# rail-berkeley/serl

Hardware: AMD Instinct MI355X
Metric: learner grad-steps/sec (DrQ, bs256, 2x128x128 img) (higher is better)
Workload: dtype f32 (trunk convs as split-fp16 MFMA x3, fp32 accumulate; <=1e-6 vs fp64)

## Files before the change

serl_amd/csrc/agent.hip:

```cpp
#include <algorithm>
#include <cmath>
#include <cstdlib>
#include <cstring>
#include <string>
#include <vector>

#include "heads.h"
#include "small_encoder.h"

using namespace serl;

namespace {

struct CamOff { long sle, dW, db, lng, lnb, conv; };
struct Offs {
  CamOff cam[SERL_MAX_CAMS];
  long cam_stride;
  long c_w1, c_b1, c_g1, c_be1, c_w2, c_b2, c_g2, c_be2, c_hw, c_hb;
  long p_W, p_b, p_g, p_be;
  long a_w1, a_b1, a_g1, a_be1, a_w2, a_b2, a_g2, a_be2, a_Wm, a_bm, a_Ws, a_bs;
  long lam;
  long P, Pc, Pa0, Pa1;
};

// ... 1223 lines not shown
  const TrunkPlan& p = a->tws.plan;
  std::string s = "images=" + std::to_string(p.images) + " pool=" + std::to_string(p.pool) + " raw_b0=" + std::to_string(p.raw_b0);
  static const char* kNames[3] = {"conv0", "conv1", "proj"};
  for (int i = 0; i < kTrunkStages; ++i)
    for (int k = 0; k < 3; ++k) {
      const TrunkPlan::L& l = p.conv[i][k];
      if (!l.kern) continue;
      s += " b" + std::to_string(i) + "_" + kNames[k] + "=" + std::string(1, l.kern) + "/" + std::to_string(l.cfg) + "/" +
           std::to_string(l.pmode) + "/f" + std::to_string(l.fused) + "/p" + std::to_string(l.pad) + "x" + std::to_string(l.padw);
    }
  SERL_REQUIRE((int)s.size() < cap, "the plan text takes %d bytes, the buffer holds %d", (int)s.size() + 1, cap);
  snprintf(out, cap, "%s", s.c_str());
  return SERL_OK;
}

int serl_agent_debug_get(serl_agent* a, const char* what, float* host_out, int64_t count) {
  SERL_REQUIRE(a && what && host_out, "NULL argument");
  SERL_HIP(hipSetDevice(a->cfg.device));
  const Offs& o = a->o;
  const std::string w(what);
  const float* p = nullptr;
  long n = 0;
  const serl_agent_cfg& c = a->cfg;
  if (w == "ctr_nonzero") {
    SERL_REQUIRE(count == 1, "tap 'ctr_nonzero' holds one value");
    SERL_HIP(hipDeviceSynchronize());
    std::vector<int> h((size_t)kCtrPerLane * kCtrLanes);
    SERL_HIP(hipMemcpy(h.data(), a->ctr, sizeof(int) * h.size(), hipMemcpyDeviceToHost));
    long nz = 0;
    for (int v : h) nz += v != 0;
    host_out[0] = (float)nz;
    return SERL_OK;
  }
  if (w == "g_critic") { p = a->Gc; n = o.Pc; }
  else if (w == "g_actor") { p = a->Ga; n = o.Pa1 - o.Pa0; }
  else if (w == "scalars") { p = a->SC; n = kScalars; }
  else if (w == "q") { p = a->crit.q; n = (long)c.ensemble * c.batch; }
  else if (w == "q_target") { p = a->critT.q; n = (long)c.ensemble * c.batch; }
  else if (w == "target_q") { p = a->ytgt; n = c.batch; }
  else if (w == "x") { p = a->crit.x; n = (long)c.batch * a->XA; }
  else if (w == "x_target") { p = a->critT.x; n = (long)c.batch * a->XA; }
  else if (w == "feats") { p = a->feats; n = 2L * c.n_cam * c.batch * a->HW * 512; }
  else if (w == "logp") { p = a->pol.logp; n = c.batch; }
  else if (w == "dx") { p = a->dx; n = (long)c.batch * a->XA; }
  else { set_error("unknown debug tap '%s'", what); return SERL_ERR_INVALID; }
  SERL_REQUIRE(count <= n && count > 0, "tap '%s' holds %ld floats, asked for %lld", what, n, (long long)count);
  SERL_HIP(hipDeviceSynchronize());
  SERL_HIP(hipMemcpy(host_out, p, sizeof(float) * count, hipMemcpyDeviceToHost));
  return SERL_OK;
}

int serl_agent_debug_set(serl_agent* a, const char* what, const float* host, int64_t count) {
  SERL_REQUIRE(a && what && host, "NULL argument");
  SERL_HIP(hipSetDevice(a->cfg.device));
  const Offs& o = a->o;
  const std::string w(what);
  float* p = nullptr;
  long n = 0;
  if (w == "g_critic") { p = a->Gc; n = o.Pc; }
  else if (w == "g_actor") { p = a->Ga; n = o.Pa1 - o.Pa0; }
  else if (w == "scalars") { p = a->SC; n = kScalars; }
  else { set_error("unknown debug tap '%s'", what); return SERL_ERR_INVALID; }
  SERL_REQUIRE(count <= n && count > 0, "tap '%s' holds %ld floats, got %lld", what, n, (long long)count);
  SERL_HIP(hipDeviceSynchronize());
  SERL_HIP(hipMemcpy(p, host, sizeof(float) * count, hipMemcpyHostToDevice));
  if (a->last_global <= 0) a->last_global = 1;
  return SERL_OK;
}

// ... 2 lines not shown
```

serl_amd/csrc/trunk.hip:

```cpp
#include <algorithm>

#include "internal.h"
#include "prof.h"
#include "trunk_common.h"

namespace serl {

struct ConvInitArgs {
  const uint8_t* img;
  const float* w;
  float* out;
  double* stats;
  int N, H, W, Ho, Wo, tiles_y, tiles_x;
};

constexpr int kCiPatch = 37;
constexpr int kCiPW = kCiPatch * 3 + 2;
constexpr int kCiK = 148;
constexpr int kCiBS = 64 + 4;

__global__ __launch_bounds__(256) void conv_init_kernel(ConvInitArgs a) {
  extern __shared__ __attribute__((aligned(16))) float smem[];
  float* patch = smem;
  float* wl = smem + kCiPatch * kCiPW + 3;
// ... 516 lines not shown
  uint8_t* b = (uint8_t*)mem;
  size_t off = 0;
  for (int i = 0; i < kTrunkStages; ++i)
    for (int k = 0; k < 3; ++k) {
      if (k == 2 && i == 0) continue;
      int K, Cout;
      conv_dims(i, k, K, Cout);
      p.blk[i][k].hi = (uint16_t*)(b + off); off += al256((size_t)K * Cout * 2);
      p.blk[i][k].lo = (uint16_t*)(b + off); off += al256((size_t)K * Cout * 2);
      p.blk[i][k].inv = (float*)(b + off); off += al256((size_t)Cout * 4);
      p.blk[i][k].dma = nullptr;
      if (dma_copy(i, k)) { p.blk[i][k].dma = (uint16_t*)(b + off); off += al256((size_t)2 * K * Cout * 2); }
    }
  p.init.hi = (uint16_t*)(b + off); off += al256((size_t)64 * 224 * 2);
  p.init.lo = (uint16_t*)(b + off); off += al256((size_t)64 * 224 * 2);
  p.init.inv = (float*)(b + off); off += al256(64 * 4);
  p.zero = b + off; off += 256;
  p.dirty = true;
  return SERL_OK;
}

static int trunk_pack(const TrunkWeights& w, TrunkPacked& p, hipStream_t stream) {
  for (int i = 0; i < kTrunkStages; ++i)
    for (int k = 0; k < 3; ++k) {
      const float* src = k == 0 ? w.blk[i].conv0 : (k == 1 ? w.blk[i].conv1 : w.blk[i].proj);
      if (!src) continue;
      int K, Cout;
      conv_dims(i, k, K, Cout);
      int rc = pack_conv_weights_f16x3(src, p.blk[i][k].hi, p.blk[i][k].lo, p.blk[i][k].inv, K, Cout, stream);
      if (rc) return rc;
      if (p.blk[i][k].dma && (rc = pack_dma_order_f16x3(p.blk[i][k].hi, p.blk[i][k].lo, p.blk[i][k].dma, K, Cout, stream))) return rc;
    }
  {
    int rc = pack_conv_init_f16x3(w.conv_init, p.init.hi, p.init.lo, p.init.inv, stream);
    if (rc) return rc;
  }
  p.dirty = false;
  return SERL_OK;
}

int trunk_forward(const TrunkWeights& w, TrunkWorkspace& ws, const uint8_t* frames, int n, float* feats_out,
                  hipStream_t stream, TrunkPacked* packed, int stage_begin, int stage_end) {
  if (packed && packed->dirty) {
    int prc = trunk_pack(w, *packed, stream);
    if (prc) return prc;
  }
  if (packed) {
    SERL_REQUIRE(n > 0 && n <= ws.max_images, "trunk_forward: %d images exceeds workspace (%d)", n, ws.max_images);
    return trunk_forward_f16x3(w, ws, *packed, frames, n, feats_out, stream, stage_begin, stage_end);
  }
  SERL_REQUIRE(stage_begin < 0 && stage_end == kTrunkStages - 1, "the exact-fp32 trunk runs whole passes only");
  SERL_REQUIRE(n > 0 && n <= ws.max_images, "trunk_forward: %d images exceeds workspace (%d)", n, ws.max_images);
  const TrunkDims& d = ws.d;
  const int N = n;
  auto stats_of = [&](int layer) { return ws.stats + (size_t)layer * ws.max_images * kGnGroups * 2; };
  SERL_HIP(hipMemsetAsync(ws.stats, 0, (size_t)kGnLayers * ws.max_images * kGnGroups * 2 * sizeof(double), stream));
  int rc;
  {
    ConvInitArgs a{};
    a.img = frames; a.w = w.conv_init; a.out = ws.raw_init; a.stats = stats_of(0);
    a.N = N; a.H = d.H; a.W = d.W; a.Ho = d.h[0]; a.Wo = d.w[0];
    a.tiles_y = cd(a.Ho, 16); a.tiles_x = cd(a.Wo, 16);
    const size_t lds = (size_t)(kCiPatch * kCiPW + 3 + kCiK * kCiBS) * 4;
    ProfScope prof("conv_init", stream);
    hipLaunchKernelGGL(conv_init_kernel, dim3(N * a.tiles_y * a.tiles_x), dim3(256), lds, stream, a);
    SERL_HIP(hipGetLastError());
  }
// ... 41 lines not shown
```

serl_amd/csrc/trunk_common.h:

```cpp
#pragma once
#include "internal.h"

namespace serl {

typedef float f32x16 __attribute__((ext_vector_type(16)));

__device__ __forceinline__ int pool_pad_lo(int in, int out) { return max((out - 1) * 2 + 3 - in, 0) >> 1; }

__device__ __forceinline__ int xcd_remap(int b, int nwg) {
  const int q = nwg >> 3, r = nwg & 7, xcd = b & 7;
  return (xcd < r ? xcd * (q + 1) : r * (q + 1) + (xcd - r) * q) + (b >> 3);
}

__device__ __forceinline__ void stats_flush(float s, float q, double* stats_ng ,
                                            int chan, int gsize, bool valid, bool wait = true) {
#pragma unroll
  for (int off = 1; off < 16; off <<= 1) {
    s += __shfl_xor(s, off);
    q += __shfl_xor(q, off);
  }
  s += __shfl_xor(s, 32);
  q += __shfl_xor(q, 32);
  const int lane = threadIdx.x & 63;
  if (valid && (lane & 15) == 0 && lane < 32) {
// ... 30 lines not shown

__device__ __forceinline__ void gn_coef4(const GnRef& g, int n, int c, float4& sc, float4& sh) {
  const double* st = g.stats + ((size_t)n * kGnGroups + c / g.gsize) * 2;
  const double mean = st[0] * g.inv_count, m2 = st[1] * g.inv_count;
  const float var = fmaxf((float)(m2 - mean * mean), 0.f);
  const float rstd = rsqrtf(var + 1e-5f), mf = (float)mean;
  const float4 ga = *reinterpret_cast<const float4*>(g.gamma + c);
  const float4 be = *reinterpret_cast<const float4*>(g.beta + c);
  sc = make_float4(ga.x * rstd, ga.y * rstd, ga.z * rstd, ga.w * rstd);
  sh = make_float4(be.x - mf * sc.x, be.y - mf * sc.y, be.z - mf * sc.z, be.w - mf * sc.w);
}

struct ConvArgs {
  const float* in;
  const float* w;
  float* out;
  double* stats;
  GnRef in_gn;
  int N, Hi, Wi, Cin, Ho, Wo, Cout, KH, KW, stride, pad, padw;
  int M, P, tiles_m, tiles_n;
};

struct PackedConvWeights {
  const uint16_t* hi;
  const uint16_t* lo;
  const float* inv;
  const uint16_t* dma = nullptr;
};
int pack_conv_weights_f16x3(const float* w, uint16_t* hi, uint16_t* lo, float* inv, int K, int Cout, hipStream_t stream);
int pack_dma_order_f16x3(const uint16_t* hi, const uint16_t* lo, uint16_t* dma, int K, int Cout, hipStream_t stream);
int trunk_forward_f16x3(const TrunkWeights& w, TrunkWorkspace& ws, TrunkPacked& pk, const uint8_t* frames, int N,
                        float* feats_out, hipStream_t stream, int stage_begin = -1, int stage_end = kTrunkStages - 1);

int pack_conv_init_f16x3(const float* w, uint16_t* hi, uint16_t* lo, float* inv, hipStream_t stream);
int launch_conv_init_f16x3(const uint8_t* img, PackedConvWeights w, float* out, double* stats, int N, int H, int W,
                           int Ho, int Wo, hipStream_t stream, const float* pool_gamma = nullptr, int* ticket = nullptr,
                           bool complete_pool = false);

}
```

serl_amd/csrc/trunk_f16x3.hip:

```cpp
#include "trunk_f16x3_elementwise.h"

namespace serl {

static int resident_workgroups(hipStream_t stream) {
  thread_local hipStream_t last = nullptr;
  thread_local int last_n = -1;
  if (last_n >= 0 && last == stream) return last_n;
  int dev = 0, n = 0;
  hipDeviceProp_t prop;
  if (hipGetDevice(&dev) == hipSuccess && hipGetDeviceProperties(&prop, dev) == hipSuccess) n = prop.multiProcessorCount;
  uint32_t mask[16] = {0};
  if (hipExtStreamGetCUMask(stream, 16, mask) == hipSuccess) {
    int m = 0;
    for (uint32_t w : mask) m += __builtin_popcount(w);
    if (m > 0 && (n == 0 || m < n)) n = m;
  } else {
    (void)hipGetLastError();
  }
  last = stream; last_n = n;
  return n;
}

static_assert(kStageFilters[0] % 64 == 0 && kStageFilters[1] % 64 == 0 && kStageFilters[2] % 64 == 0 && kStageFilters[3] % 64 == 0,
              "conv channels unsupported (Cin % 32, Cout % 64)");
// ... 28 lines not shown
  const bool dma_ok = (cfg == 0 || cfg == 4) && a.Cin % 32 == 0 && zero_page && dma && fits32;
  if (slab_ok) {
    l.kern = 'S'; l.cfg = 9; l.raw = raw;
    const int tiles_n = a.Cout / 64;
    if (fuse && a.P % 256 == 0 && fused_can_wait(resident, a.P / 256 * tiles_n)) {
      l.fused = 1; l.expected = a.P / 256; l.group = a.P / 256 * tiles_n;
    }
    l.stagger = (l.fused && a.M / 256 * tiles_n >= 1024) ? 5 : 0;
  } else if (dma_ok) {
    l.kern = 'D'; l.cfg = cfg;
    const int tn = cfg == 0 ? 2 : 1, tiles_n = a.Cout / (64 * tn);
    if (pmode == 1 && cfg == 4) pmode = 3;
    if (fuse && pmode == 0 && a.P % 128 == 0 && tiles_n <= kSyncPerImage && fused_can_wait(resident, a.P / 128 * tiles_n)) {
      l.fused = 1; l.expected = a.P / 128; l.group = a.P / 128 * tiles_n;
    } else if (fuse && pmode == 0 && a.P == 64 && a.M % 128 == 0 && tn == 2 && a.Cout / kGnGroups == 64) {
      l.fused = 2;
    } else if (fuse && pmode == 2 && a.P == 16 && a.M % 128 == 0 && tn == 2 && a.Cout / kGnGroups == 128) {
      l.fused = 2;
    }
    l.proj = proj && pmode != 3 && a.KH == 3 && a.stride == 2 && a.pad == 0 && a.padw == 0;
  } else {
    l.kern = 'R'; l.cfg = cfg;
  }
  l.pmode = pmode;
  l.pad = a.pad; l.padw = a.padw;
  return l;
}

static int plan_pass(TrunkPlan& p, const TrunkDims& d, int N, const TrunkPacked& pk, const bool (&has_proj)[kTrunkStages], int resident,
                     bool fuse, bool proj_fuse) {
  p = TrunkPlan{};
  p.images = N; p.fuse = fuse;
  const bool fuse_pool = d.h[0] % 16 == 0 && d.w[0] % 16 == 0;
  const bool complete_pool = fuse_pool && N >= 512 && N % 512 == 0;
  p.pool = complete_pool ? 2 : (fuse_pool ? 1 : 0);
  const ConvArgs b0 = conv_geom(d, N, 0, 0);
  p.raw_b0 = complete_pool && fuse && !has_proj[0] && rowslab_shape_ok(b0) && b0.Cin <= 128 && pk.blk[0][0].dma && pk.blk[0][1].dma &&
             b0.P % 256 == 0 && fused_can_wait(resident, b0.P / 256 * (b0.Cout / 64));
  for (int i = 0; i < kTrunkStages; ++i) {
    TrunkPlan::L* l = p.conv[i];
    const bool raw = i == 0 && p.raw_b0;
    l[0] = plan_conv(conv_geom(d, N, i, 0), pk.blk[i][0].dma, pk.zero, fuse, resident, raw, has_proj[i] && proj_fuse && pk.blk[i][2].dma);
    if (l[0].proj) {
      l[2] = l[0];
      l[2].kern = 'F'; l[2].fused = 0;
    } else if (has_proj[i]) {
      l[2] = plan_conv(conv_geom(d, N, i, 2), pk.blk[i][2].dma, pk.zero, false, resident, false, false);
    }
    l[1] = plan_conv(conv_geom(d, N, i, 1), pk.blk[i][1].dma, pk.zero, fuse, resident, false, false);
    SERL_REQUIRE(!raw || (l[0].kern == 'S' && l[0].fused && l[1].fused),
                 "block 0 was planned on the fused row-slab path");
  }
  return SERL_OK;
}

template <int WM, int WN, int TM, int TN, int DEEP>
static void launch_igemm(ConvArgsB ab, int pmode, hipStream_t stream) {
  constexpr int BM = 32 * TM * WM, BN = 32 * TN * WN;
  ab.c.tiles_m = cdiv(ab.c.M, BM); ab.c.tiles_n = ab.c.Cout / BN;
  const dim3 grid(ab.c.tiles_m * ab.c.tiles_n), block(256);
  const size_t lds = (size_t)2 * (2 * BM * 64 + 2 * BN * 64);
  if (pmode == 0) hipLaunchKernelGGL((conv_igemm_f16x3_kernel<WM, WN, TM, TN, 0, DEEP>), grid, block, lds, stream, ab);
  else if (pmode == 1) hipLaunchKernelGGL((conv_igemm_f16x3_kernel<WM, WN, TM, TN, 1, DEEP>), grid, block, lds, stream, ab);
  else if (pmode == 2) hipLaunchKernelGGL((conv_igemm_f16x3_kernel<WM, WN, TM, TN, 2, DEEP>), grid, block, lds, stream, ab);
  else hipLaunchKernelGGL((conv_igemm_f16x3_kernel<WM, WN, TM, TN, 3, DEEP>), grid, block, lds, stream, ab);
}
template <int TN, bool PROJ>
// ... 76 lines not shown
                        float* feats_out, hipStream_t stream, int stage_begin, int stage_end) {
  const TrunkDims& d = ws.d;
  const TrunkPlan& plan = ws.plan;
  auto stats_of = [&](int layer) { return ws.stats + (size_t)layer * ws.max_images * kGnGroups * 2; };
  int rc;
  if (stage_begin < 0) {
    const char* gf = getenv("SERL_GN_FUSE");
    const char* pf = getenv("SERL_PROJ_FUSE");
    const bool fuse = !(gf && gf[0] == '0') && claim_fused_pass(stream);
    const bool has_proj[kTrunkStages] = {w.blk[0].proj != nullptr, w.blk[1].proj != nullptr, w.blk[2].proj != nullptr,
                                         w.blk[3].proj != nullptr};
    const int resident = fuse ? resident_workgroups(stream) : 0;
    if ((rc = plan_pass(ws.plan, d, N, pk, has_proj, resident, fuse, !(pf && pf[0] == '0')))) return rc;
    if (ws.stats_sync_bytes % 16 == 0 && ws.stats_sync_bytes < ((size_t)1 << 31)) {
      const long n16 = (long)(ws.stats_sync_bytes / 16);
      hipLaunchKernelGGL(zero_sys_kernel, dim3((unsigned)std::min<long>(cdiv(n16, 256), 512)), dim3(256), 0, stream, (void*)ws.stats, n16);
      SERL_HIP(hipGetLastError());
    } else {
      SERL_HIP(hipMemsetAsync(ws.stats, 0, ws.stats_sync_bytes, stream));
    }
  } else {
    SERL_REQUIRE(plan.images == N, "trunk pass piece over %d images continues a pass planned for %d", N, plan.images);
  }
  auto fuse_of = [&](int layer, int mode) {
    FuseArgs f{};
    f.mode = mode;
    f.sync = ws.sync + (size_t)layer * ((size_t)ws.max_images * kSyncPerImage + kSyncTickets);
    f.ticket = f.sync + (size_t)ws.max_images * kSyncPerImage;
    return f;
  };
  const GnRef gn_init = gn_ref(stats_of(0), w.gn_init_s, w.gn_init_b, d.h[0] * d.w[0], 64);
  if (stage_begin < 0) {
    if ((rc = launch_conv_init_f16x3(frames, PackedConvWeights{pk.init.hi, pk.init.lo, pk.init.inv}, ws.raw_init, stats_of(0), N, d.H,
                                     d.W, d.h[0], d.w[0], stream, plan.pool ? w.gn_init_s : nullptr, fuse_of(0, 0).ticket,
                                     plan.pool == 2))) return rc;
    if (plan.raw_b0) {
    } else if (plan.pool == 2) {
      const long tot = (long)N * d.h[1] * d.w[1] * 16;
      ProfScope prof("gn_relu_maxpool", stream);
      hipLaunchKernelGGL(gn_relu_split_kernel, dim3(cdiv(tot, 256)), dim3(256), 0, stream, ws.raw_init, gn_init,
                         reinterpret_cast<uint4*>(ws.pool), N, d.h[1] * d.w[1], 64);
      SERL_HIP(hipGetLastError());
    } else if (plan.pool == 1) {
      const long tot = (long)N * d.h[1] * (d.w[1] / 4) * 16;
      const int ty = d.h[0] / 16, tx = d.w[0] / 16;
      const float* pooled = ws.raw_init;
      const float* frows = pooled + (size_t)N * d.h[1] * d.w[1] * 64;
      const float* fcols = frows + (size_t)N * ty * d.w[0] * 64;
      ProfScope prof("gn_relu_maxpool", stream);
      hipLaunchKernelGGL(pool_finish_split_kernel, dim3(cdiv(tot, 256)), dim3(256), 0, stream, pooled, frows, fcols, gn_init,
                         reinterpret_cast<uint4*>(ws.pool), N, d.h[0], d.w[0], ty, tx);
      SERL_HIP(hipGetLastError());
    } else {
      const long tot = (long)N * d.h[1] * d.w[1] * 16;
      ProfScope prof("gn_relu_maxpool", stream);
      hipLaunchKernelGGL(gn_relu_maxpool_split_kernel, dim3(cdiv(tot, 256)), dim3(256), 0, stream, ws.raw_init, gn_init,
                         reinterpret_cast<uint4*>(ws.pool), N, d.h[0], d.w[0], d.h[1], d.w[1], 64);
      SERL_HIP(hipGetLastError());
    }
  }
  auto run_stage = [&](int i) -> int {
    const int f = kStageFilters[i], P = d.h[2 + i] * d.w[2 + i];
    const int l0 = 1 + 3 * i, l1 = 2 + 3 * i, lp = 3 + 3 * i;
    const TrunkWeights::Block& bw = w.blk[i];
    const TrunkWorkspace::B& t = ws.blk[i];
    const TrunkPlan::L* pl = plan.conv[i];
    const bool has_proj = bw.proj != nullptr, last = i == kTrunkStages - 1;
// ... 57 lines not shown
```

serl_amd/csrc/trunk_f16x3_conv_init.h:

```cpp
#pragma once
#include "trunk_f16x3_rowslab.h"

namespace serl {

struct ConvInitArgsB {
  const uint8_t* img;
  const uint16_t* whi;
  const uint16_t* wlo;
  const float* winv;
  float* out;
  double* stats;
  int N, H, W, Ho, Wo, tiles_y, tiles_x, total_tiles;
  const float* gamma;
  float* pooled;
  float* first_rows;
  float* first_cols;
  int chunk;
  int* ticket;
  int wprio;
};

constexpr int kCbPatch = 37;

constexpr int kC8K = 224;
constexpr int kC8WP = 232;
constexpr int kC8Pitch = 384;
constexpr int kC8WBytes = 64 * kC8WP * 2;
constexpr int kC8PBytes = 14336;
constexpr int kC8Lds = 2 * kC8WBytes + kC8PBytes;
static_assert(kCbPatch * kC8Pitch <= kC8PBytes, "patch does not fit");

template <int POOL>
__global__ __launch_bounds__(256, 2) void conv_init_u8_kernel(ConvInitArgsB a) {
  extern __shared__ __attribute__((aligned(16))) uint8_t smemb[];
  uint8_t* w_hi = smemb;
  uint8_t* w_lo = smemb + kC8WBytes;
  uint8_t* patch = smemb + 2 * kC8WBytes;
  const int tid = threadIdx.x, lane = tid & 63, wave = __builtin_amdgcn_readfirstlane(tid >> 6);
  const int li = lane & 31, lh = lane >> 5;
  if (a.wprio) __builtin_amdgcn_s_setprio(3);
  for (int v = tid; v < 2 * 64 * (kC8K / 8); v += 256) {
    const int plane = v / (64 * 28), r = (v / 28) % 64, sl = v % 28;
    const uint4 val = *reinterpret_cast<const uint4*>((plane ? a.wlo : a.whi) + (size_t)r * kC8K + sl * 8);
    *reinterpret_cast<uint4*>((plane ? w_lo : w_hi) + r * (kC8WP * 2) + sl * 16) = val;
  }
  constexpr int kGroups = 10, kTasks = kCbPatch * kGroups;
  const long img_bytes = (long)a.N * a.H * a.W * 3;
  const bool aligned = (a.W & 3) == 0 && (reinterpret_cast<uintptr_t>(a.img) & 3) == 0;
  uint32_t pre[2][3];
  unsigned pmask[2];
  const int tpi = a.tiles_y * a.tiles_x;
#define SERL_C8_ORDER(T) (POOL == 2 ? (T) - (T) % tpi + (tpi - 1 - (T) % tpi) : (T))
#define SERL_C8_FETCH(TILE)                                                                             \
  {                                                                                                     \
    int b_ = SERL_C8_ORDER(TILE);                                                                       \
    const int tx_ = b_ % a.tiles_x;                                                                     \
    b_ /= a.tiles_x;                                                                                    \
    const int ty_ = b_ % a.tiles_y;                                                                     \
    const int n_ = b_ / a.tiles_y;                                                                      \
    _Pragma("unroll") for (int q = 0; q < 2; ++q) {                                                     \
      const int t_ = tid + 256 * q;                                                                     \
      const int r_ = t_ / kGroups, g_ = t_ - r_ * kGroups;                                              \
      const int iy = ty_ * 32 - 3 + r_, ixg = tx_ * 32 - 4 + 4 * g_;                                    \
      const bool rowok = t_ < kTasks && (unsigned)iy < (unsigned)a.H;                                   \
      unsigned m_ = 0;                                                                                  \
      _Pragma("unroll") for (int j = 0; j < 4; ++j)                                                     \
        if (rowok && (unsigned)(ixg + j) < (unsigned)a.W) m_ |= 1u << j;                                \
      pmask[q] = m_;                                                                                    \
      long off_ = (((long)n_ * a.H + min(max(iy, 0), a.H - 1)) * a.W + ixg) * 3;                        \
      if (aligned) {                                                                                    \
        _Pragma("unroll") for (int d = 0; d < 3; ++d) {                                                 \
          const long o_ = min(max(off_ + 4 * d, 0L), img_bytes - 4);                                    \
          pre[q][d] = *reinterpret_cast<const uint32_t*>(a.img + o_);       \
        }                                                                                               \
      } else {                                                                                          \
        _Pragma("unroll") for (int d = 0; d < 3; ++d) {                                                 \
          uint32_t w_ = 0;                                                                              \
          _Pragma("unroll") for (int e = 0; e < 4; ++e) {                                               \
            const long o_ = min(max(off_ + 4 * d + e, 0L), img_bytes - 1);                              \
            w_ |= (uint32_t)a.img[o_] << (8 * e);                                                       \
          }                                                                                             \
          pre[q][d] = w_;                                                                               \
        }                                                                                               \
      }                                                                                                 \
    }                                                                                                   \
  }
  __shared__ int s_next_chunk;
  const int nchunks = a.total_tiles / a.chunk;
  float s[2] = {0.f, 0.f}, q[2] = {0.f, 0.f};
  const float winv[2] = {a.winv[li], a.winv[32 + li]};
  float sgn[2] = {1.f, 1.f};
  if (POOL) { sgn[0] = a.gamma[li] < 0.f ? -1.f : 1.f; sgn[1] = a.gamma[32 + li] < 0.f ? -1.f : 1.f; }
  int chunk = blockIdx.x, next_chunk = 0;
  int tile = chunk * a.chunk, t_end = tile + a.chunk;
  if (chunk < nchunks) SERL_C8_FETCH(tile);
  while (chunk < nchunks) {
    const bool first_of_chunk = tile == chunk * a.chunk;
    if (first_of_chunk && tid == 0)
      s_next_chunk = (int)gridDim.x + __hip_atomic_fetch_add(a.ticket, 1, __ATOMIC_RELAXED, __HIP_MEMORY_SCOPE_SYSTEM);
    int b = SERL_C8_ORDER(tile);
    const int tx = b % a.tiles_x;
    b /= a.tiles_x;
    const int ty = b % a.tiles_y;
    const int n = b / a.tiles_y;
    const int oy0 = ty * 16, ox0 = tx * 16;
    __syncthreads();
#pragma unroll
    for (int q = 0; q < 2; ++q) {
      const int t = tid + 256 * q;
      if (t < kTasks) {
        const int r = t / kGroups, g = t - r * kGroups;
        const uint32_t d0 = pre[q][0], d1 = pre[q][1], d2 = pre[q][2];
        const uint32_t by[12] = {d0 & 255u, (d0 >> 8) & 255u, (d0 >> 16) & 255u, d0 >> 24, d1 & 255u, (d1 >> 8) & 255u,
                                 (d1 >> 16) & 255u, d1 >> 24, d2 & 255u, (d2 >> 8) & 255u, (d2 >> 16) & 255u, d2 >> 24};
        uint8_t* rowp = patch + r * kC8Pitch;
#pragma unroll
        for (int j = 0; j < 4; ++j) {
          const int col = 4 * g - 1 + j;
          if (col < 0) continue;
          const bool in = (pmask[q] >> j) & 1u;
          const f16x2 c01 = {(_Float16)(float)by[3 * j], (_Float16)(float)by[3 * j + 1]};
          const f16x2 c2b = {(_Float16)(float)by[3 * j + 2], (_Float16)1.0f};
          u32x2 rec = {__builtin_bit_cast(unsigned, c01), __builtin_bit_cast(unsigned, c2b)};
          if (!in) rec = (u32x2){0u, 0u};
          *reinterpret_cast<u32x2*>(rowp + col * 8) = rec;
        }
      }
    }
    __syncthreads();
    if (first_of_chunk) next_chunk = __builtin_amdgcn_readfirstlane(s_next_chunk);
    SERL_C8_FETCH(min(tile + 1 < t_end ? tile + 1 : next_chunk * a.chunk, a.total_tiles - 1));
    float nb_col[2][4], nb_row[2][4][3];
    const bool has_right = POOL == 2 && tx + 1 < a.tiles_x, has_below = POOL == 2 && ty + 1 < a.tiles_y;
    if (POOL == 2) {
      const float* dummy = reinterpret_cast<const float*>(a.whi) + li;
      {
        const float* fcn = has_right ? a.first_cols + (((size_t)n * a.Ho + oy0 + wave * 4) * a.tiles_x + tx + 1) * 64 + li : dummy;
#pragma unroll
        for (int tn = 0; tn < 2; ++tn)
#pragma unroll
          for (int i = 0; i < 4; ++i) nb_col[tn][i] = fcn[has_right ? (size_t)i * a.tiles_x * 64 + tn * 32 : (size_t)(i * 64 + tn * 32)];
      }
      if (wave == 3) {
        const float* frn = has_below ? a.first_rows + (((size_t)n * a.tiles_y + ty + 1) * a.Wo + ox0) * 64 + li : dummy;
#pragma unroll
        for (int tn = 0; tn < 2; ++tn)
#pragma unroll
          for (int sl = 0; sl < 4; ++sl) {
            const int px = 2 * (2 * (sl >> 1) + lh) + (sl & 1);
#pragma unroll
            for (int dx = 0; dx < 3; ++dx) {
              const int x = min(2 * px + dx, a.Wo - 1 - ox0);
              nb_row[tn][sl][dx] = frn[(size_t)x * 64 + tn * 32];
            }
          }
      }
    }
    int abase[2];
#pragma unroll
    for (int tm = 0; tm < 2; ++tm) {
      const int p = wave * 64 + tm * 32 + li;
      abase[tm] = (2 * (p >> 4)) * kC8Pitch + (p & 15) * 16 + lh * 16;
    }
    const int bbase = li * (kC8WP * 2) + lh * 16;
    f32x16 acc[2][2];
#pragma unroll
    for (int tm = 0; tm < 2; ++tm)
#pragma unroll
      for (int tn = 0; tn < 2; ++tn)
#pragma unroll
        for (int r = 0; r < 16; ++r) acc[tm][tn][r] = 0.f;
#pragma unroll
    for (int ks = 0; ks < kC8K / 16; ++ks) {
      const int aoff = (ks >> 1) * kC8Pitch + (ks & 1) * 32;
      f16x8 apx[2], bhi[2], blo[2];
#pragma unroll
      for (int tm = 0; tm < 2; ++tm) apx[tm] = *reinterpret_cast<const f16x8*>(patch + abase[tm] + aoff);
#pragma unroll
      for (int tn = 0; tn < 2; ++tn) {
        const int off = bbase + tn * 32 * (kC8WP * 2) + ks * 32;
        bhi[tn] = *reinterpret_cast<const f16x8*>(w_hi + off);
        blo[tn] = *reinterpret_cast<const f16x8*>(w_lo + off);
      }
#pragma unroll
      for (int tm = 0; tm < 2; ++tm)
#pragma unroll
        for (int tn = 0; tn < 2; ++tn) {
          acc[tm][tn] = __builtin_amdgcn_mfma_f32_32x32x16_f16(apx[tm], blo[tn], acc[tm][tn], 0, 0, 0);
          acc[tm][tn] = __builtin_amdgcn_mfma_f32_32x32x16_f16(apx[tm], bhi[tn], acc[tm][tn], 0, 0, 0);
        }
    }
#pragma unroll
    for (int q = 0; q < 2; ++q)
#pragma unroll
      for (int d = 0; d < 3; ++d) asm volatile("" : : "v"(pre[q][d]), "v"(acc[1][1][15]));
    if (POOL == 2) {
#pragma unroll
      for (int tn = 0; tn < 2; ++tn)
#pragma unroll
        for (int i = 0; i < 4; ++i) asm volatile("" : : "v"(nb_col[tn][i]), "v"(acc[1][1][15]));
      if (wave == 3) {
#pragma unroll
        for (int tn = 0; tn < 2; ++tn)
#pragma unroll
          for (int sl = 0; sl < 4; ++sl)
#pragma unroll
            for (int dx = 0; dx < 3; ++dx) asm volatile("" : : "v"(nb_row[tn][sl][dx]), "v"(acc[1][1][15]));
      }
    }
#pragma unroll
    for (int tm = 0; tm < 2; ++tm)
#pragma unroll
      for (int tn = 0; tn < 2; ++tn)
#pragma unroll
        for (int r = 0; r < 16; ++r) acc[tm][tn][r] *= winv[tn];
    if (POOL == 0) {
#pragma unroll
      for (int tm = 0; tm < 2; ++tm)
#pragma unroll
        for (int r = 0; r < 16; ++r) {
          const int p = wave * 64 + tm * 32 + (r & 3) + 8 * (r >> 2) + 4 * lh;
          const int oy = oy0 + (p >> 4), ox = ox0 + (p & 15);
          const bool ok = oy < a.Ho && ox < a.Wo;
          float* o = a.out + (((size_t)n * a.Ho + oy) * a.Wo + ox) * 64;
#pragma unroll
          for (int tn = 0; tn < 2; ++tn) {
            const float v = ok ? acc[tm][tn][r] : 0.f;
            if (ok) o[tn * 32 + li] = v;
            s[tn] += v;
            q[tn] += v * v;
          }
        }
    } else {
#pragma unroll
      for (int tm = 0; tm < 2; ++tm)
#pragma unroll
        for (int r = 0; r < 16; ++r)
#pragma unroll
          for (int tn = 0; tn < 2; ++tn) {
            const float v = acc[tm][tn][r];
            s[tn] += v;
            q[tn] += v * v;
          }
      if (wave == 0) {
        float* fr = a.first_rows + (((size_t)n * a.tiles_y + (oy0 >> 4)) * a.Wo + ox0 + 4 * lh) * 64 + li;
#pragma unroll
        for (int r = 0; r < 8; ++r)
#pragma unroll
          for (int tn = 0; tn < 2; ++tn) fr[(8 * (r >> 2) + (r & 3)) * 64 + tn * 32] = acc[0][tn][r];
      }
      if (lh == 0) {
        float* fc = a.first_cols + (((size_t)n * a.Ho + oy0 + wave * 4) * a.tiles_x + (ox0 >> 4)) * 64 + li;
#pragma unroll
        for (int tm = 0; tm < 2; ++tm)
#pragma unroll
          for (int rr = 0; rr < 2; ++rr)
#pragma unroll
            for (int tn = 0; tn < 2; ++tn)
              fc[(size_t)(tm * 2 + rr) * a.tiles_x * 64 + tn * 32] = acc[tm][tn][8 * rr];
      }
      float hrow[2][4][4];
#pragma unroll
      for (int tn = 0; tn < 2; ++tn) {
        const float sg = sgn[tn];
#pragma unroll
        for (int i = 0; i < 4; ++i) {
          float part[2], v0[2];
#pragma unroll
          for (int qd = 0; qd < 2; ++qd) {
            const int rb = 8 * (i & 1) + 4 * qd;
            const float c0 = sg * acc[i >> 1][tn][rb], c1 = sg * acc[i >> 1][tn][rb + 1];
            const float c2 = sg * acc[i >> 1][tn][rb + 2], c3 = sg * acc[i >> 1][tn][rb + 3];
            hrow[tn][i][2 * qd] = fmaxf(fmaxf(c0, c1), c2);
            part[qd] = fmaxf(c2, c3);
            v0[qd] = c0;
          }
          const float r0 = __shfl_xor(v0[0], 32), r1 = __shfl_xor(v0[1], 32);
          hrow[tn][i][1] = fmaxf(part[0], lh ? r1 : r0);
          hrow[tn][i][3] = lh ? part[1] : fmaxf(part[1], r1);
          if (POOL == 2 && has_right && lh) hrow[tn][i][3] = fmaxf(hrow[tn][i][3], sg * nb_col[tn][i]);
        }
      }
      __syncthreads();
      float* ex = reinterpret_cast<float*>(patch);
#pragma unroll
      for (int tn = 0; tn < 2; ++tn)
#pragma unroll
        for (int sl = 0; sl < 4; ++sl) ex[((wave * 2 + tn) * 4 + sl) * 64 + lane] = hrow[tn][0][sl];
      __syncthreads();
      const int Hp = a.Ho >> 1, Wp = a.Wo >> 1;
#pragma unroll
      for (int tn = 0; tn < 2; ++tn) {
        const float sg = sgn[tn];
        float* orow = a.pooled + (((size_t)n * Hp + (oy0 >> 1) + 2 * wave) * Wp + (ox0 >> 1)) * 64 + tn * 32 + li;
#pragma unroll
        for (int sl = 0; sl < 4; ++sl) {
          const int px = 2 * (2 * (sl >> 1) + lh) + (sl & 1);
          const float even = fmaxf(fmaxf(hrow[tn][0][sl], hrow[tn][1][sl]), hrow[tn][2][sl]);
          float odd = fmaxf(hrow[tn][2][sl], hrow[tn][3][sl]);
          if (wave < 3) odd = fmaxf(odd, ex[(((wave + 1) * 2 + tn) * 4 + sl) * 64 + lane]);
          else if (POOL == 2 && has_below)
            odd = fmaxf(odd, fmaxf(fmaxf(sg * nb_row[tn][sl][0], sg * nb_row[tn][sl][1]), sg * nb_row[tn][sl][2]));
          orow[(size_t)px * 64] = sg * even;
          orow[((size_t)Wp + px) * 64] = sg * odd;
        }
      }
    }
    if (++tile == t_end) {
      double* st = a.stats + (size_t)n * kGnGroups * 2;
#pragma unroll
      for (int tn = 0; tn < 2; ++tn) stats_flush(s[tn], q[tn], st, tn * 32 + li, 16, true, false);
      s[0] = s[1] = q[0] = q[1] = 0.f;
      chunk = next_chunk;
      tile = chunk * a.chunk;
      t_end = tile + a.chunk;
    }
  }
#undef SERL_C8_FETCH
#undef SERL_C8_ORDER
}

__device__ __forceinline__ float channel_scale(float m, int top, float* red ) {
#pragma unroll
  for (int off = 32; off > 0; off >>= 1) m = fmaxf(m, __shfl_xor(m, off));
  if ((threadIdx.x & 63) == 0) red[threadIdx.x >> 6] = m;
  __syncthreads();
  m = fmaxf(fmaxf(red[0], red[1]), fmaxf(red[2], red[3]));
  __syncthreads();
  if (!(m > 0.f) || !(m < 3.0e38f)) return 1.0f;
  int e;
  frexpf(m, &e);
  return ldexpf(1.0f, min(max(top - e, -100), 100));
}

__global__ __launch_bounds__(256) void pack_conv_init_u8_kernel(const float* w, uint16_t* hi, uint16_t* lo, float* inv) {
  __shared__ float red[4];
  const int n = blockIdx.x, kp = threadIdx.x;
  const int ky = kp >> 5, kx = (kp >> 2) & 7, ln = kp & 3;
  const double mean[3] = {0.485, 0.456, 0.406}, stdv[3] = {0.229, 0.224, 0.225};
  double v = 0.0;
  if (kp < kC8K && kx < 7) {
    if (ln < 3) v = (double)w[(size_t)(ky * 21 + kx * 3 + ln) * 64 + n] / (255.0 * stdv[ln]);
    else
      for (int c = 0; c < 3; ++c) v -= (double)w[(size_t)(ky * 21 + kx * 3 + c) * 64 + n] * (mean[c] / stdv[c]);
  }
  const float sc = channel_scale(fabsf((float)v), 13, red);
  if (kp == 0) inv[n] = 1.0f / sc;
  if (kp >= kC8K) return;
  const float vs = (float)(v * (double)sc);
  const _Float16 h = (_Float16)clamp_h(vs);
  const _Float16 l = (_Float16)(vs - (float)h);
  hi[(size_t)n * kC8K + kp] = __builtin_bit_cast(uint16_t, h);
  lo[(size_t)n * kC8K + kp] = __builtin_bit_cast(uint16_t, l);
}

int pack_conv_init_f16x3(const float* w, uint16_t* hi, uint16_t* lo, float* inv, hipStream_t stream) {
  static_assert(kC8K <= 256, "one thread per k'");
  hipLaunchKernelGGL(pack_conv_init_u8_kernel, dim3(64), dim3(256), 0, stream, w, hi, lo, inv);
  SERL_HIP(hipGetLastError());
  return SERL_OK;
}

int launch_conv_init_f16x3(const uint8_t* img, PackedConvWeights w, float* out, double* stats, int N, int H, int W,
                           int Ho, int Wo, hipStream_t stream, const float* pool_gamma, int* ticket, bool complete_pool) {
  ConvInitArgsB a{};
  a.img = img; a.whi = w.hi; a.wlo = w.lo; a.winv = w.inv; a.out = out; a.stats = stats;
  a.N = N; a.H = H; a.W = W; a.Ho = Ho; a.Wo = Wo;
  a.wprio = trunk_wave_prio(N);
  a.tiles_y = cdiv(Ho, 16); a.tiles_x = cdiv(Wo, 16);
  a.total_tiles = N * a.tiles_y * a.tiles_x;
  SERL_REQUIRE(ticket != nullptr, "conv_init needs a chunk ticket");
  const int tpi = a.tiles_y * a.tiles_x;
  a.chunk = (pool_gamma && complete_pool) ? tpi : (tpi % 4 == 0 ? 4 : (tpi % 2 == 0 ? 2 : 1));
  a.ticket = ticket;
  const int grid = std::min(a.total_tiles / a.chunk, 512);
  ProfScope prof("conv_init", stream);
  if (pool_gamma) {
    SERL_REQUIRE(Ho % 16 == 0 && Wo % 16 == 0, "fused conv_init pooling needs full 16x16 tiles");
    a.gamma = pool_gamma;
    a.pooled = out;
    a.first_rows = a.pooled + (size_t)N * (Ho / 2) * (Wo / 2) * 64;
    a.first_cols = a.first_rows + (size_t)N * a.tiles_y * Wo * 64;
    if (complete_pool) hipLaunchKernelGGL(conv_init_u8_kernel<2>, dim3(grid), dim3(256), kC8Lds, stream, a);
    else hipLaunchKernelGGL(conv_init_u8_kernel<1>, dim3(grid), dim3(256), kC8Lds, stream, a);
  } else {
    hipLaunchKernelGGL(conv_init_u8_kernel<0>, dim3(grid), dim3(256), kC8Lds, stream, a);
  }
  SERL_HIP(hipGetLastError());
  return SERL_OK;
}

}
```

Baseline: 437.9.

## Keep conv_init pooling halos in registers and fold gamma sign into packed weights

```diff
diff --git a/serl_amd/csrc/agent.hip b/serl_amd/csrc/agent.hip
--- a/serl_amd/csrc/agent.hip
+++ b/serl_amd/csrc/agent.hip
@@ -1279,9 +1279,24 @@
     host_out[0] = (float)nz;
     return SERL_OK;
   }
+  if (w == "trunk_stats0") {
+    const long nd = (long)a->tws.plan.images * kGnGroups * 2;
+    SERL_REQUIRE(!a->state_only && !a->small && nd > 0 && count == 2 * nd, "tap 'trunk_stats0' holds %ld floats, asked for %lld", 2 * nd, (long long)count);
+    SERL_HIP(hipDeviceSynchronize());
+    std::vector<double> h((size_t)nd);
+    SERL_HIP(hipMemcpy(h.data(), a->tws.stats, sizeof(double) * h.size(), hipMemcpyDeviceToHost));
+    for (long i = 0; i < nd; ++i) {
+      host_out[2 * i] = (float)h[i];
+      host_out[2 * i + 1] = (float)(h[i] - (double)host_out[2 * i]);
+    }
+    return SERL_OK;
+  }
   if (w == "g_critic") { p = a->Gc; n = o.Pc; }
   else if (w == "g_actor") { p = a->Ga; n = o.Pa1 - o.Pa0; }
   else if (w == "scalars") { p = a->SC; n = kScalars; }
+  else if (w == "trunk_pooled_raw" && !a->state_only && !a->small && a->tws.plan.pool == 2) {
+    p = a->tws.raw_init; n = (long)a->tws.plan.images * a->tws.d.h[1] * a->tws.d.w[1] * 64;
+  }
   else if (w == "q") { p = a->crit.q; n = (long)c.ensemble * c.batch; }
   else if (w == "q_target") { p = a->critT.q; n = (long)c.ensemble * c.batch; }
   else if (w == "target_q") { p = a->ytgt; n = c.batch; }
diff --git a/serl_amd/csrc/trunk.hip b/serl_amd/csrc/trunk.hip
--- a/serl_amd/csrc/trunk.hip
+++ b/serl_amd/csrc/trunk.hip
@@ -572,7 +572,7 @@
       if (p.blk[i][k].dma && (rc = pack_dma_order_f16x3(p.blk[i][k].hi, p.blk[i][k].lo, p.blk[i][k].dma, K, Cout, stream))) return rc;
     }
   {
-    int rc = pack_conv_init_f16x3(w.conv_init, p.init.hi, p.init.lo, p.init.inv, stream);
+    int rc = pack_conv_init_f16x3(w.conv_init, w.gn_init_s, p.init.hi, p.init.lo, p.init.inv, stream);
     if (rc) return rc;
   }
   p.dirty = false;
diff --git a/serl_amd/csrc/trunk_common.h b/serl_amd/csrc/trunk_common.h
--- a/serl_amd/csrc/trunk_common.h
+++ b/serl_amd/csrc/trunk_common.h
@@ -86,9 +86,9 @@
 int trunk_forward_f16x3(const TrunkWeights& w, TrunkWorkspace& ws, TrunkPacked& pk, const uint8_t* frames, int N,
                         float* feats_out, hipStream_t stream, int stage_begin = -1, int stage_end = kTrunkStages - 1);
 
-int pack_conv_init_f16x3(const float* w, uint16_t* hi, uint16_t* lo, float* inv, hipStream_t stream);
+int pack_conv_init_f16x3(const float* w, const float* gamma, uint16_t* hi, uint16_t* lo, float* inv, hipStream_t stream);
 int launch_conv_init_f16x3(const uint8_t* img, PackedConvWeights w, float* out, double* stats, int N, int H, int W,
-                           int Ho, int Wo, hipStream_t stream, const float* pool_gamma = nullptr, int* ticket = nullptr,
+                           int Ho, int Wo, hipStream_t stream, bool pool = false, int* ticket = nullptr,
                            bool complete_pool = false);
 
 }
diff --git a/serl_amd/csrc/trunk_f16x3.hip b/serl_amd/csrc/trunk_f16x3.hip
--- a/serl_amd/csrc/trunk_f16x3.hip
+++ b/serl_amd/csrc/trunk_f16x3.hip
@@ -84,7 +84,7 @@
   p = TrunkPlan{};
   p.images = N; p.fuse = fuse;
   const bool fuse_pool = d.h[0] % 16 == 0 && d.w[0] % 16 == 0;
-  const bool complete_pool = fuse_pool && N >= 512 && N % 512 == 0;
+  const bool complete_pool = fuse_pool && N >= 512 && N % 512 == 0 && d.w[0] <= 16 * kC8Ring;
   p.pool = complete_pool ? 2 : (fuse_pool ? 1 : 0);
   const ConvArgs b0 = conv_geom(d, N, 0, 0);
   p.raw_b0 = complete_pool && fuse && !has_proj[0] && rowslab_shape_ok(b0) && b0.Cin <= 128 && pk.blk[0][0].dma && pk.blk[0][1].dma &&
@@ -227,7 +227,7 @@
   const GnRef gn_init = gn_ref(stats_of(0), w.gn_init_s, w.gn_init_b, d.h[0] * d.w[0], 64);
   if (stage_begin < 0) {
     if ((rc = launch_conv_init_f16x3(frames, PackedConvWeights{pk.init.hi, pk.init.lo, pk.init.inv}, ws.raw_init, stats_of(0), N, d.H,
-                                     d.W, d.h[0], d.w[0], stream, plan.pool ? w.gn_init_s : nullptr, fuse_of(0, 0).ticket,
+                                     d.W, d.h[0], d.w[0], stream, plan.pool != 0, fuse_of(0, 0).ticket,
                                      plan.pool == 2))) return rc;
     if (plan.raw_b0) {
     } else if (plan.pool == 2) {
diff --git a/serl_amd/csrc/trunk_f16x3_conv_init.h b/serl_amd/csrc/trunk_f16x3_conv_init.h
--- a/serl_amd/csrc/trunk_f16x3_conv_init.h
+++ b/serl_amd/csrc/trunk_f16x3_conv_init.h
@@ -11,7 +11,6 @@
   float* out;
   double* stats;
   int N, H, W, Ho, Wo, tiles_y, tiles_x, total_tiles;
-  const float* gamma;
   float* pooled;
   float* first_rows;
   float* first_cols;
@@ -30,6 +29,8 @@
 constexpr int kC8Lds = 2 * kC8WBytes + kC8PBytes;
 static_assert(kCbPatch * kC8Pitch <= kC8PBytes, "patch does not fit");
 
+constexpr int kC8Ring = 4;
+static_assert((4 * 2 + 2) * 4 * 64 * 4 <= kC8PBytes, "five row-exchange slots fit the patch buffer");
 template <int POOL>
 __global__ __launch_bounds__(256, 2) void conv_init_u8_kernel(ConvInitArgsB a) {
   extern __shared__ __attribute__((aligned(16))) uint8_t smemb[];
@@ -89,11 +90,20 @@
   const int nchunks = a.total_tiles / a.chunk;
   float s[2] = {0.f, 0.f}, q[2] = {0.f, 0.f};
   const float winv[2] = {a.winv[li], a.winv[32 + li]};
-  float sgn[2] = {1.f, 1.f};
-  if (POOL) { sgn[0] = a.gamma[li] < 0.f ? -1.f : 1.f; sgn[1] = a.gamma[32 + li] < 0.f ? -1.f : 1.f; }
+  float pcol[2][4] = {}, ring[kC8Ring][2][4] = {};
+  unsigned rmask[kC8Ring];
+#pragma unroll
+  for (int k = 0; k < kC8Ring; ++k) rmask[k] = __builtin_amdgcn_readfirstlane(a.tiles_x - 1 == k ? ~0u : 0u);
   int chunk = blockIdx.x, next_chunk = 0;
   int tile = chunk * a.chunk, t_end = tile + a.chunk;
-  if (chunk < nchunks) SERL_C8_FETCH(tile);
+  if (chunk < nchunks) {
+    SERL_C8_FETCH(tile);
+#pragma unroll
+    for (int q = 0; q < 2; ++q)
+#pragma unroll
+      for (int d = 0; d < 3; ++d) asm volatile("" : : "v"(pre[q][d]));
+  }
+  asm volatile("" : : "v"(winv[0]), "v"(winv[1]));
   while (chunk < nchunks) {
     const bool first_of_chunk = tile == chunk * a.chunk;
     if (first_of_chunk && tid == 0)
@@ -130,32 +140,7 @@
     __syncthreads();
     if (first_of_chunk) next_chunk = __builtin_amdgcn_readfirstlane(s_next_chunk);
     SERL_C8_FETCH(min(tile + 1 < t_end ? tile + 1 : next_chunk * a.chunk, a.total_tiles - 1));
-    float nb_col[2][4], nb_row[2][4][3];
     const bool has_right = POOL == 2 && tx + 1 < a.tiles_x, has_below = POOL == 2 && ty + 1 < a.tiles_y;
-    if (POOL == 2) {
-      const float* dummy = reinterpret_cast<const float*>(a.whi) + li;
-      {
-        const float* fcn = has_right ? a.first_cols + (((size_t)n * a.Ho + oy0 + wave * 4) * a.tiles_x + tx + 1) * 64 + li : dummy;
-#pragma unroll
-        for (int tn = 0; tn < 2; ++tn)
-#pragma unroll
-          for (int i = 0; i < 4; ++i) nb_col[tn][i] = fcn[has_right ? (size_t)i * a.tiles_x * 64 + tn * 32 : (size_t)(i * 64 + tn * 32)];
-      }
-      if (wave == 3) {
-        const float* frn = has_below ? a.first_rows + (((size_t)n * a.tiles_y + ty + 1) * a.Wo + ox0) * 64 + li : dummy;
-#pragma unroll
-        for (int tn = 0; tn < 2; ++tn)
-#pragma unroll
-          for (int sl = 0; sl < 4; ++sl) {
-            const int px = 2 * (2 * (sl >> 1) + lh) + (sl & 1);
-#pragma unroll
-            for (int dx = 0; dx < 3; ++dx) {
-              const int x = min(2 * px + dx, a.Wo - 1 - ox0);
-              nb_row[tn][sl][dx] = frn[(size_t)x * 64 + tn * 32];
-            }
-          }
-      }
-    }
     int abase[2];
 #pragma unroll
     for (int tm = 0; tm < 2; ++tm) {
@@ -194,26 +179,6 @@
     for (int q = 0; q < 2; ++q)
 #pragma unroll
       for (int d = 0; d < 3; ++d) asm volatile("" : : "v"(pre[q][d]), "v"(acc[1][1][15]));
-    if (POOL == 2) {
-#pragma unroll
-      for (int tn = 0; tn < 2; ++tn)
-#pragma unroll
-        for (int i = 0; i < 4; ++i) asm volatile("" : : "v"(nb_col[tn][i]), "v"(acc[1][1][15]));
-      if (wave == 3) {
-#pragma unroll
-        for (int tn = 0; tn < 2; ++tn)
-#pragma unroll
-          for (int sl = 0; sl < 4; ++sl)
-#pragma unroll
-            for (int dx = 0; dx < 3; ++dx) asm volatile("" : : "v"(nb_row[tn][sl][dx]), "v"(acc[1][1][15]));
-      }
-    }
-#pragma unroll
-    for (int tm = 0; tm < 2; ++tm)
-#pragma unroll
-      for (int tn = 0; tn < 2; ++tn)
-#pragma unroll
-        for (int r = 0; r < 16; ++r) acc[tm][tn][r] *= winv[tn];
     if (POOL == 0) {
 #pragma unroll
       for (int tm = 0; tm < 2; ++tm)
@@ -225,7 +190,7 @@
           float* o = a.out + (((size_t)n * a.Ho + oy) * a.Wo + ox) * 64;
 #pragma unroll
           for (int tn = 0; tn < 2; ++tn) {
-            const float v = ok ? acc[tm][tn][r] : 0.f;
+            const float v = ok ? acc[tm][tn][r] * winv[tn] : 0.f;
             if (ok) o[tn * 32 + li] = v;
             s[tn] += v;
             q[tn] += v * v;
@@ -242,14 +207,14 @@
             s[tn] += v;
             q[tn] += v * v;
           }
-      if (wave == 0) {
+      if (POOL == 1 && wave == 0) {
         float* fr = a.first_rows + (((size_t)n * a.tiles_y + (oy0 >> 4)) * a.Wo + ox0 + 4 * lh) * 64 + li;
 #pragma unroll
         for (int r = 0; r < 8; ++r)
 #pragma unroll
-          for (int tn = 0; tn < 2; ++tn) fr[(8 * (r >> 2) + (r & 3)) * 64 + tn * 32] = acc[0][tn][r];
-      }
-      if (lh == 0) {
+          for (int tn = 0; tn < 2; ++tn) fr[(8 * (r >> 2) + (r & 3)) * 64 + tn * 32] = acc[0][tn][r] * winv[tn];
+      }
+      if (POOL == 1 && lh == 0) {
         float* fc = a.first_cols + (((size_t)n * a.Ho + oy0 + wave * 4) * a.tiles_x + (ox0 >> 4)) * 64 + li;
 #pragma unroll
         for (int tm = 0; tm < 2; ++tm)
@@ -257,20 +222,19 @@
           for (int rr = 0; rr < 2; ++rr)
 #pragma unroll
             for (int tn = 0; tn < 2; ++tn)
-              fc[(size_t)(tm * 2 + rr) * a.tiles_x * 64 + tn * 32] = acc[tm][tn][8 * rr];
+              fc[(size_t)(tm * 2 + rr) * a.tiles_x * 64 + tn * 32] = acc[tm][tn][8 * rr] * winv[tn];
       }
       float hrow[2][4][4];
 #pragma unroll
       for (int tn = 0; tn < 2; ++tn) {
-        const float sg = sgn[tn];
 #pragma unroll
         for (int i = 0; i < 4; ++i) {
           float part[2], v0[2];
 #pragma unroll
           for (int qd = 0; qd < 2; ++qd) {
             const int rb = 8 * (i & 1) + 4 * qd;
-            const float c0 = sg * acc[i >> 1][tn][rb], c1 = sg * acc[i >> 1][tn][rb + 1];
-            const float c2 = sg * acc[i >> 1][tn][rb + 2], c3 = sg * acc[i >> 1][tn][rb + 3];
+            const float c0 = acc[i >> 1][tn][rb], c1 = acc[i >> 1][tn][rb + 1];
+            const float c2 = acc[i >> 1][tn][rb + 2], c3 = acc[i >> 1][tn][rb + 3];
             hrow[tn][i][2 * qd] = fmaxf(fmaxf(c0, c1), c2);
             part[qd] = fmaxf(c2, c3);
             v0[qd] = c0;
@@ -278,38 +242,60 @@
           const float r0 = __shfl_xor(v0[0], 32), r1 = __shfl_xor(v0[1], 32);
           hrow[tn][i][1] = fmaxf(part[0], lh ? r1 : r0);
           hrow[tn][i][3] = lh ? part[1] : fmaxf(part[1], r1);
-          if (POOL == 2 && has_right && lh) hrow[tn][i][3] = fmaxf(hrow[tn][i][3], sg * nb_col[tn][i]);
+          if (POOL == 2) {
+            hrow[tn][i][3] = fmaxf(hrow[tn][i][3], has_right && lh ? pcol[tn][i] : hrow[tn][i][3]);
+            pcol[tn][i] = r0;
+          }
         }
       }
       __syncthreads();
       float* ex = reinterpret_cast<float*>(patch);
+      float below[2][4];
 #pragma unroll
       for (int tn = 0; tn < 2; ++tn)
 #pragma unroll
-        for (int sl = 0; sl < 4; ++sl) ex[((wave * 2 + tn) * 4 + sl) * 64 + lane] = hrow[tn][0][sl];
+        for (int sl = 0; sl < 4; ++sl) {
+          ex[((wave * 2 + tn) * 4 + sl) * 64 + lane] = hrow[tn][0][sl];
+          if (POOL == 2) {
+            unsigned bits = 0;
+#pragma unroll
+            for (int k = 0; k < kC8Ring; ++k) bits |= __builtin_bit_cast(unsigned, ring[k][tn][sl]) & rmask[k];
+            below[tn][sl] = __builtin_bit_cast(float, bits);
+#pragma unroll
+            for (int k = kC8Ring - 1; k > 0; --k) ring[k][tn][sl] = ring[k - 1][tn][sl];
+            ring[0][tn][sl] = hrow[tn][0][sl];
+          }
+        }
+      if (POOL == 2 && wave == 0 && has_below) {
+#pragma unroll
+        for (int tn = 0; tn < 2; ++tn)
+#pragma unroll
+          for (int sl = 0; sl < 4; ++sl) ex[((4 * 2 + tn) * 4 + sl) * 64 + lane] = below[tn][sl];
+      }
       __syncthreads();
       const int Hp = a.Ho >> 1, Wp = a.Wo >> 1;
 #pragma unroll
       for (int tn = 0; tn < 2; ++tn) {
-        const float sg = sgn[tn];
         float* orow = a.pooled + (((size_t)n * Hp + (oy0 >> 1) + 2 * wave) * Wp + (ox0 >> 1)) * 64 + tn * 32 + li;
 #pragma unroll
         for (int sl = 0; sl < 4; ++sl) {
           const int px = 2 * (2 * (sl >> 1) + lh) + (sl & 1);
           const float even = fmaxf(fmaxf(hrow[tn][0][sl], hrow[tn][1][sl]), hrow[tn][2][sl]);
           float odd = fmaxf(hrow[tn][2][sl], hrow[tn][3][sl]);
-          if (wave < 3) odd = fmaxf(odd, ex[(((wave + 1) * 2 + tn) * 4 + sl) * 64 + lane]);
-          else if (POOL == 2 && has_below)
-            odd = fmaxf(odd, fmaxf(fmaxf(sg * nb_row[tn][sl][0], sg * nb_row[tn][sl][1]), sg * nb_row[tn][sl][2]));
-          orow[(size_t)px * 64] = sg * even;
-          orow[((size_t)Wp + px) * 64] = sg * odd;
+          if (wave < 3 || has_below)
+            odd = fmaxf(odd, ex[(((wave + 1) * 2 + tn) * 4 + sl) * 64 + lane]);
+          orow[(size_t)px * 64] = even * winv[tn];
+          orow[((size_t)Wp + px) * 64] = odd * winv[tn];
         }
       }
     }
     if (++tile == t_end) {
       double* st = a.stats + (size_t)n * kGnGroups * 2;
 #pragma unroll
-      for (int tn = 0; tn < 2; ++tn) stats_flush(s[tn], q[tn], st, tn * 32 + li, 16, true, false);
+      for (int tn = 0; tn < 2; ++tn) {
+        const float sr = POOL ? s[tn] * winv[tn] : s[tn], qr = POOL ? q[tn] * winv[tn] * winv[tn] : q[tn];
+        stats_flush(sr, qr, st, tn * 32 + li, 16, true, false);
+      }
       s[0] = s[1] = q[0] = q[1] = 0.f;
       chunk = next_chunk;
       tile = chunk * a.chunk;
@@ -333,7 +319,7 @@
   return ldexpf(1.0f, min(max(top - e, -100), 100));
 }
 
-__global__ __launch_bounds__(256) void pack_conv_init_u8_kernel(const float* w, uint16_t* hi, uint16_t* lo, float* inv) {
+__global__ __launch_bounds__(256) void pack_conv_init_u8_kernel(const float* w, const float* gamma, uint16_t* hi, uint16_t* lo, float* inv) {
   __shared__ float red[4];
   const int n = blockIdx.x, kp = threadIdx.x;
   const int ky = kp >> 5, kx = (kp >> 2) & 7, ln = kp & 3;
@@ -345,24 +331,26 @@
       for (int c = 0; c < 3; ++c) v -= (double)w[(size_t)(ky * 21 + kx * 3 + c) * 64 + n] * (mean[c] / stdv[c]);
   }
   const float sc = channel_scale(fabsf((float)v), 13, red);
-  if (kp == 0) inv[n] = 1.0f / sc;
+  const float sg = gamma[n] < 0.f ? -1.f : 1.f;
+  if (kp == 0) inv[n] = sg / sc;
   if (kp >= kC8K) return;
-  const float vs = (float)(v * (double)sc);
+  const float vs = sg * (float)(v * (double)sc);
   const _Float16 h = (_Float16)clamp_h(vs);
   const _Float16 l = (_Float16)(vs - (float)h);
   hi[(size_t)n * kC8K + kp] = __builtin_bit_cast(uint16_t, h);
   lo[(size_t)n * kC8K + kp] = __builtin_bit_cast(uint16_t, l);
 }
 
-int pack_conv_init_f16x3(const float* w, uint16_t* hi, uint16_t* lo, float* inv, hipStream_t stream) {
+int pack_conv_init_f16x3(const float* w, const float* gamma, uint16_t* hi, uint16_t* lo, float* inv, hipStream_t stream) {
   static_assert(kC8K <= 256, "one thread per k'");
-  hipLaunchKernelGGL(pack_conv_init_u8_kernel, dim3(64), dim3(256), 0, stream, w, hi, lo, inv);
+  SERL_REQUIRE(gamma != nullptr, "conv_init's packed weights carry the sign of norm_init's scale");
+  hipLaunchKernelGGL(pack_conv_init_u8_kernel, dim3(64), dim3(256), 0, stream, w, gamma, hi, lo, inv);
   SERL_HIP(hipGetLastError());
   return SERL_OK;
 }
 
 int launch_conv_init_f16x3(const uint8_t* img, PackedConvWeights w, float* out, double* stats, int N, int H, int W,
-                           int Ho, int Wo, hipStream_t stream, const float* pool_gamma, int* ticket, bool complete_pool) {
+                           int Ho, int Wo, hipStream_t stream, bool pool, int* ticket, bool complete_pool) {
   ConvInitArgsB a{};
   a.img = img; a.whi = w.hi; a.wlo = w.lo; a.winv = w.inv; a.out = out; a.stats = stats;
   a.N = N; a.H = H; a.W = W; a.Ho = Ho; a.Wo = Wo;
@@ -371,13 +359,13 @@
   a.total_tiles = N * a.tiles_y * a.tiles_x;
   SERL_REQUIRE(ticket != nullptr, "conv_init needs a chunk ticket");
   const int tpi = a.tiles_y * a.tiles_x;
-  a.chunk = (pool_gamma && complete_pool) ? tpi : (tpi % 4 == 0 ? 4 : (tpi % 2 == 0 ? 2 : 1));
+  a.chunk = (pool && complete_pool) ? tpi : (tpi % 4 == 0 ? 4 : (tpi % 2 == 0 ? 2 : 1));
   a.ticket = ticket;
   const int grid = std::min(a.total_tiles / a.chunk, 512);
   ProfScope prof("conv_init", stream);
-  if (pool_gamma) {
+  if (pool) {
     SERL_REQUIRE(Ho % 16 == 0 && Wo % 16 == 0, "fused conv_init pooling needs full 16x16 tiles");
-    a.gamma = pool_gamma;
+    SERL_REQUIRE(!complete_pool || a.tiles_x <= kC8Ring, "complete conv_init pooling keeps %d tiles' first rows, not %d", kC8Ring, a.tiles_x);
     a.pooled = out;
     a.first_rows = a.pooled + (size_t)N * (Ho / 2) * (Wo / 2) * 64;
     a.first_cols = a.first_rows + (size_t)N * a.tiles_y * Wo * 64;
```

New measurement: 435.0. About the same (-0.7%).
